# syun88/VLA-from-FastVLM

Hardware: AMD Instinct MI355X
Metric: policy steps/sec (img+prompt->action) FastVLM-0.5B bs=64 (higher is better)
Workload: dtype bf16; 1 GPU; fastvlm-0.5b select_action: letterbox 336^2->1024^2, FastViT-HD, projector, Qwen2 decoder (text-only, reference-literal: 64-token prompt), last-token pool, action head; batch_per_gpu=64, global_batch=64, seq_len=64, image=336, parallelism=replicas x1 (no collective on the inference path), tower_microbatch=0, stream_overlap=True, llm_precision=split-bf16 (hi+lo) operands, fp32 attention

## Files before the change

### vla-from-fastvlm_amd/csrc/decoder_kernels.hip

```cpp
#include "kernels.h"

namespace fv {
#define FV_TRY_RC(expr) do { const int rc_ = (expr); if (rc_ != FV_OK) return rc_; } while (0)
namespace {

__global__ __launch_bounds__(256) void embed_gather_kernel(const int32_t* __restrict__ ids,
                                                            const bf16_t* __restrict__ table,
                                                            const float* __restrict__ img, float* __restrict__ x, int T,
                                                            int Ni, int H, int vocab, long rows) {
  const int lane = threadIdx.x & 63;
  const long row = (long)blockIdx.x * 4 + (threadIdx.x >> 6);
  if (row >= rows) return;
  const int Tt = Ni + T;
  const long b = row / Tt;
  const int t = (int)(row % Tt);
  float* dst = x + row * H;
  if (t < Ni) {
    const float* src = img + (b * Ni + t) * H;
    for (int i = lane * 4; i < H; i += 256) *reinterpret_cast<float4*>(dst + i) = *reinterpret_cast<const float4*>(src + i);
  } else {
    int id = ids[b * T + (t - Ni)];
    id = min(max(id, 0), vocab - 1);
    const bf16_t* src = table + (size_t)id * H;
    for (int i = lane * 8; i < H; i += 512) {
// ... 353 lines not shown
  const float denom = mode == 0 ? 1.0f : fmaxf((float)(r1 - r0), 1e-6f);
  for (int i = tid; i < H; i += 256) pooled[(size_t)b * H + i] = 0.f;
  for (int r = r0; r < r1; ++r) {
    const float* xr = x + ((size_t)b * Ttot + r) * H;
    float ss = 0.f;
    for (int i = tid; i < H; i += 256) ss += xr[i] * xr[i];
    ss = wave_sum(ss);
    __syncthreads();
    if ((tid & 63) == 0) red[tid >> 6] = ss;
    __syncthreads();
    const float rs = rsqrtf((red[0] + red[1] + red[2] + red[3]) / (float)H + eps);
    for (int i = tid; i < H; i += 256) pooled[(size_t)b * H + i] += w[i] * (xr[i] * rs) / denom;
  }
}

}

int launch_embed_gather(const int32_t* ids, const bf16_t* table, const float* img_tokens, float* x, int B, int T,
                        int Ni, int H, int vocab, hipStream_t s) {
  if (!ids || !table || !x) return fv_fail(FV_ERR_ARG, "embed_gather: null pointer");
  if (Ni > 0 && !img_tokens) return fv_fail(FV_ERR_ARG, "embed_gather: Ni > 0 without image tokens");
  if (B <= 0 || T <= 0 || Ni < 0 || H % 8 || vocab <= 0) return fv_fail(FV_ERR_ARG, "embed_gather: bad shape");
  const long rows = (long)B * (Ni + T);
  hipLaunchKernelGGL(embed_gather_kernel, dim3((unsigned)((rows + 3) / 4)), dim3(256), 0, s, ids, table, img_tokens, x, T, Ni, H, vocab, rows);
  FV_HIP_CHECK(hipGetLastError());
  return FV_OK;
}

int launch_rmsnorm(const float* x, const float* w, bf16_t* y, bf16_t* y_lo, int ldy, int rows, int H, float eps, hipStream_t s, int f16, unsigned* sat, int lo8) {
  if (!x || !w || !y) return fv_fail(FV_ERR_ARG, "rmsnorm: null pointer");
// ... 149 lines not shown
```

### vla-from-fastvlm_amd/csrc/engine.hip

```cpp
#include <dlfcn.h>

#include <algorithm>
#include <exception>
#include <climits>
#include <cmath>
#include <new>
#include <cstdarg>
#include <cstdio>
#include <cstdlib>
#include <cstring>
#include <functional>
#include <map>
#include <string>
#include <vector>

#include "kernels.h"

static thread_local char g_err[768] = "";
static thread_local char* g_err_handle = nullptr;
int fv_fail(int code, const char* fmt, ...) {
  va_list ap;
  va_start(ap, fmt);
  vsnprintf(g_err, sizeof(g_err), fmt, ap);
  va_end(ap);
// ... 584 lines not shown
  }
  const int CL = d.tower_dims[d.tower_stages - 1], CO = d.tower_out_dim, P = H * H;
  FV_P(FV_FAM_DWCONV, dw_flops(mb, H, H, CO, 3), 2.0 * mb * P * (CL + CO), fv::launch_dwconv(cur, tw.exp_w, tw.exp_b, oth, mb, H, H, CL, 3, 1, CO / CL, 0, s));
  FV_P(FV_FAM_ELT, 20.0 * mb * P * CO, 6.0 * mb * P * CO, fv::launch_se_gelu(oth, tw.se_w1, tw.se_b1, tw.se_w2, tw.se_b2, tower_out, se, mb, P, CO, d.tower_se_rd, s));
  fv::GemmArgs p0{tower_out, CO, tw.pj0_w, mb * P, d.llm_hidden, CO, tw.pj0_b, nullptr, nullptr, 0, hid, d.llm_hidden, FV_EPI_BIAS_GELU};
  if (!h->batch_invariant) { p0.splitk_ws = h->ffn_part; p0.splitk_bytes = h->ffn_part ? FFN_PART_BYTES : 0; }
  FV_TRY(gemm_p(h, p0, s));
  fv::GemmArgs p2{hid, d.llm_hidden, tw.pj2_w, mb * P, d.llm_hidden, d.llm_hidden, tw.pj2_b, nullptr, nullptr, 0, img_tokens, d.llm_hidden, FV_EPI_F32};
  FV_TRY(gemm_p(h, p2, s));
  return FV_OK;
}


enum DecMode { DEC_FULL = 0, DEC_PREFIX = 1, DEC_SUFFIX = 2 };
int decoder_layers_split(fv_handle* h, const WsPlan& wp, int B, int Tq, const int32_t* lens, int len_add, float* kv, int Np, int mode,
                         hipStream_t s) {
  const fv_model_desc& d = h->d;
  char* ws = static_cast<char*>(h->ws);
  float* x = reinterpret_cast<float*>(ws + wp.x);
  bf16_t* xn = reinterpret_cast<bf16_t*>(ws + wp.xn);
  bf16_t* act = reinterpret_cast<bf16_t*>(ws + wp.act);
  const int rows = B * Tq, Hd = d.llm_hidden, D = d.llm_head_dim;
  const int qd = d.llm_heads * D, kd = d.llm_kv_heads * D, qkvw = qd + 2 * kd;
  const int Tt = mode == DEC_SUFFIX ? Np + Tq : Tq;
  const float att_scale = 1.0f / std::sqrt((float)D);
  {
    bf16_t* xs = reinterpret_cast<bf16_t*>(ws + wp.xn_lo);
    bf16_t* as = reinterpret_cast<bf16_t*>(ws + wp.att_lo);
    bf16_t* cs = reinterpret_cast<bf16_t*>(ws + wp.act_lo);
    float* qkvf = reinterpret_cast<float*>(ws + wp.qkvf);
    const int I = d.llm_inter, I2 = 2 * I;
// ... 4 lines not shown
      if (li == 0) FV_P(FV_FAM_NORM, 4.0 * rows * Hd, 8.0 * rows * Hd, fv::launch_rmsnorm(x, L.ln1, xs, xs + Hd, 2 * Hd, rows, Hd, d.rms_eps, s, 0, nullptr, lo8));
      fv::GemmArgs q1{xs, 2 * Hd, L.qkv_w, rows, qkvw, Hd, L.qkv_b, nullptr, nullptr, 0, qkvf, qkvw, FV_EPI_F32, KS};
      q1.W8 = L.qkv_w8;
      q1.splitk_ws = wp.splitk_bytes ? reinterpret_cast<float*>(ws + wp.splitk) : nullptr;
      q1.splitk_bytes = wp.splitk_bytes;
      FV_TRY(gemm_p(h, q1, s));
      if (mode == DEC_PREFIX) {
        FV_HIP_CHECK(hipMemcpy2DAsync(kv + li * kv_layer, (size_t)2 * kd * 4, qkvf + qd, (size_t)qkvw * 4, (size_t)2 * kd * 4, (size_t)rows,
                                      hipMemcpyDeviceToDevice, s));
        if (li + 1 == h->dec.layers.size()) break;
      }
      FV_P(FV_FAM_ATTN, 2.0 * B * (double)Tq * Tt * qd + 3.0 * rows * (qd + kd), 4.0 * rows * (qkvw + qd),
           fv::launch_attention_f32(qkvf, qkvw, as, as + qd, 2 * qd, B, Tt, d.llm_heads, d.llm_kv_heads, D, lens, len_add, att_scale, s, h->rope,
                                    mode == DEC_SUFFIX ? kv + li * kv_layer : nullptr, 2 * kd, mode == DEC_SUFFIX ? Np : 0, nullptr, lo8,
                                    wp.attn_scr_bytes && mode != DEC_SUFFIX ? ws + wp.attn_scr : nullptr));
      fv::GemmArgs o1{as, 2 * qd, L.o_w, rows, Hd, qd, nullptr, nullptr, x, Hd, x, Hd, FV_EPI_RES_F32, KS};
      o1.W8 = L.o_w8;
      o1.splitk_ws = q1.splitk_ws;
      o1.splitk_bytes = wp.splitk_bytes;
      const bool ln2_fused = d.llm_precision == 1 || d.llm_precision == 5;
      if (ln2_fused) { o1.norm_w = L.ln2; o1.norm_y = xs; o1.norm_ylo = xs + Hd; o1.norm_ld = 2 * Hd; o1.norm_eps = d.rms_eps; }
      FV_TRY(gemm_p(h, o1, s));
      fv::GemmArgs d1{cs, I2, L.down_w, rows, Hd, I, nullptr, nullptr, x, Hd, x, Hd, FV_EPI_RES_F32, KS};
      d1.W8 = L.down_w8;
      if (d.llm_precision == 2) {
        FV_P(FV_FAM_NORM, 4.0 * rows * Hd, 6.0 * rows * Hd, fv::launch_rmsnorm(x, L.ln2, xn, nullptr, Hd, rows, Hd, d.rms_eps, s, 1, h->f16_flags));
        fv::GemmArgs g1{xn, Hd, L.gu_w, rows, I2, Hd, nullptr, nullptr, nullptr, 0, act, I, FV_EPI_SWIGLU_F16, 0};
        g1.f16 = 1; g1.sat = h->f16_flags;
        FV_TRY(gemm_p(h, g1, s));
        d1 = fv::GemmArgs{act, I, L.down_w, rows, Hd, I, nullptr, nullptr, x, Hd, x, Hd, FV_EPI_RES_F32, 0};
// ... 414 lines not shown
      fv::GemmArgs gq{xn, Hd, L.qkv_w, rows, qkvw, Hd, L.qkv_b, nullptr, nullptr, 0, qkv, qkvw, FV_EPI_BIAS};
      FV_TRY(gemm_p(h, gq, s));
      FV_P(FV_FAM_ELT, 3.0 * rows * (qd + kd), 4.0 * rows * (qd + kd), fv::launch_rope(qkv, h->rope, qkvw, rows, Tt, d.llm_heads, d.llm_kv_heads, D, s));
      FV_P(FV_FAM_ATTN, 2.0 * B * (double)Tt * Tt * qd, 2.0 * rows * (qkvw + qd),
           fv::launch_attention(qkv, qkv + qd, qkv + qd + kd, qkvw, qkvw, qkvw, att, qd, B, Tt, d.llm_heads, d.llm_kv_heads,
                                D, 1, lens, Ni, att_scale, s));
      fv::GemmArgs go{att, qd, L.o_w, rows, Hd, qd, nullptr, nullptr, x, Hd, x, Hd, FV_EPI_RES_F32};
      FV_TRY(gemm_p(h, go, s));
      FV_P(FV_FAM_NORM, 4.0 * rows * Hd, 6.0 * rows * Hd, fv::launch_rmsnorm(x, L.ln2, xn, nullptr, Hd, rows, Hd, d.rms_eps, s));
      fv::GemmArgs gg{xn, Hd, L.gu_w, rows, 2 * d.llm_inter, Hd, nullptr, nullptr, nullptr, 0, act, d.llm_inter, FV_EPI_SWIGLU};
      FV_TRY(gemm_p(h, gg, s));
      fv::GemmArgs gd{act, d.llm_inter, L.down_w, rows, Hd, d.llm_inter, nullptr, nullptr, x, Hd, x, Hd, FV_EPI_RES_F32};
      FV_TRY(gemm_p(h, gd, s));
    }
  } else {
    FV_TRY(decoder_layers_split(h, wp, B, Tt, lens, Ni, nullptr, 0, DEC_FULL, s));
  }
  FV_P(FV_FAM_ELT, 4.0 * B * Hd, 8.0 * B * Hd, fv::launch_pool_norm(x, lens, h->dec.norm, static_cast<float*>(pooled), B, Tt, Ni, Hd, d.rms_eps, pool_mode, s));
  return FV_OK;
}

int fv_set_batch_invariant(fv_handle* h, int on) {
  HandleScope _hs(h);
  if (!h) return fv_fail(FV_ERR_ARG, "fv_set_batch_invariant: null handle");
  h->batch_invariant = on != 0;
  return FV_OK;
}

int fv_llm_fp16_saturations(fv_handle* h, uint64_t* count_out, int reset) {
  HandleScope _hs(h);
  if (!h || !count_out) return fv_fail(FV_ERR_ARG, "fv_llm_fp16_saturations: null argument");
// ... 33 lines not shown
                                   int pool_mode, void* pooled, fv_stream st) {
  HandleScope _hs(h);
  FV_TRY(check_ready(h, true));
  if (!ids || !lens || !kv || !pooled || B <= 0 || T <= 0 || Ni <= 0) return fv_fail(FV_ERR_ARG, "fv_llm_forward_pooled_prefixed: bad argument");
  const fv_model_desc& d = h->d;
  if (d.llm_precision == 0 || d.llm_head_dim < 64) return fv_fail(FV_ERR_UNSUPPORTED, "fv_llm_forward_pooled_prefixed: needs llm_precision 1 / 2 and head_dim 64 / 128");
  if (pool_mode != 0) return fv_fail(FV_ERR_UNSUPPORTED, "fv_llm_forward_pooled_prefixed: mean_pool averages the image positions too, which this pass does not recompute");
  if (T + Ni > h->rope_rows) return fv_fail(FV_ERR_ARG, "sequence of %d tokens exceeds the RoPE table (%d)", T + Ni, h->rope_rows);
  if (B > d.max_batch) return fv_fail(FV_ERR_ARG, "B=%d exceeds max_batch=%d", B, d.max_batch);
  const WsPlan wp = plan_ws(h, B, T, 1);
  if (wp.total > h->ws_bytes) return fv_fail(FV_ERR_STATE, "workspace too small (%zu > %zu)", wp.total, h->ws_bytes);
  hipStream_t s = static_cast<hipStream_t>(st);
  float* x = reinterpret_cast<float*>(static_cast<char*>(h->ws) + wp.x);
  const int Hd = d.llm_hidden;
  FV_P(FV_FAM_ELT, 0.0, 6.0 * B * T * Hd, fv::launch_embed_gather(ids, h->dec.embed, nullptr, x, B, T, 0, Hd, d.llm_vocab, s));
  FV_TRY(decoder_layers_split(h, wp, B, T, lens, Ni, const_cast<float*>(static_cast<const float*>(kv)), Ni, DEC_SUFFIX, s));
  FV_P(FV_FAM_ELT, 4.0 * B * Hd, 8.0 * B * Hd, fv::launch_pool_norm(x, lens, h->dec.norm, static_cast<float*>(pooled), B, T, 0, Hd, d.rms_eps, 0, s));
  return FV_OK;
}

int fv_head_layout(fv_handle* h, int64_t offsets[13]) {
  HandleScope _hs(h);
  if (!h || !offsets) return fv_fail(FV_ERR_ARG, "fv_head_layout: null argument");
  const fv::HeadOffsets ho = fv::head_offsets(h->hd);
  for (int i = 0; i < 13; ++i) offsets[i] = ho.o[i];
  return FV_OK;
}

int fv_head_saved_bytes(fv_handle* h, int B, size_t* out_bytes) {
  HandleScope _hs(h);
  if (!h || !out_bytes || B <= 0) return fv_fail(FV_ERR_ARG, "fv_head_saved_bytes: bad argument");
  *out_bytes = fv::head_saved_bytes(h->hd, B);
// ... 286 lines not shown
```

### vla-from-fastvlm_amd/csrc/gemm_bf16.hip

```cpp
#include <cstdlib>
#include <type_traits>

#include "kernels.h"

namespace fv {
namespace {

constexpr int BN = 128, BK = 64;
constexpr int LDC = BN + 4;

struct Params {
  const bf16_t* A; const bf16_t* W; const float* bias; const float* scale; const void* res; void* out;
  int M, N, K, lda, ldr, ldo, epi, tiles_n, nwg, ksplit;
  int splits = 1, npad = 0; float* part = nullptr;
  int lo_off = 0;
  int tiles_m = 0;
  int group_m = 0, tiles_mt = 0;
  int ldw = 0;
  const uint8_t* W8 = nullptr;
  unsigned* sat = nullptr;
  void* stash = nullptr;
  int stash_f16 = 0;
};

// ... 283 lines not shown
#define G2_T(I) { const unsigned long long n_ = __builtin_readcyclecounter(); st_[I] += n_ - t0_; t0_ = n_; }
#else
#define G2_T(I)
#endif
typedef __attribute__((address_space(3))) void* lds_ptr_t;
typedef const __attribute__((address_space(1))) void* gptr_t;
typedef __attribute__((ext_vector_type(4))) short g2_s16x4;
__device__ __forceinline__ bf16x8 g2_tr_frag(const char* region, int cols16, int c16, int ks, uint32_t tr_lane, int fq_hi) {
  const char* p0 = region + ((((4 * ks + fq_hi) * (cols16 >> 2) + (c16 >> 2)) << 10) + (((c16 >> 1) & 1) << 9) + ((c16 & 1) << 5) + tr_lane);
  const g2_s16x4 lo = __builtin_amdgcn_ds_read_tr16_b64_v4i16((g2_s16x4 __attribute__((address_space(3)))*)(p0));
  const g2_s16x4 hi = __builtin_amdgcn_ds_read_tr16_b64_v4i16((g2_s16x4 __attribute__((address_space(3)))*)(p0 + ((2 * (cols16 >> 2)) << 10)));
  const uint2 lu = __builtin_bit_cast(uint2, lo), hu = __builtin_bit_cast(uint2, hi);
  return __builtin_bit_cast(bf16x8, make_uint4(lu.x, lu.y, hu.x, hu.y));
}

template <int MI, int WN, bool ASYM = false, bool F16 = false, bool LO8 = false, bool TN = false>
__global__ __launch_bounds__(128 * WN, WN == 4 ? 1 : 2) void gemm256_kernel(Params p) {
  static_assert(!ASYM || WN == 4, "asymmetric staging pairs wave w with wave w + 4");
  static_assert(!TN || (!ASYM && !LO8 && MI == 8 && WN == 4), "the TN instance is the plain 256 x 256 one");
  constexpr int BMT = 32 * MI, BNT = 64 * WN, NTH = 128 * WN, BUFB = (BMT + BNT) * 128, AB = BMT * 128;
  constexpr int SA = BMT * 8 / NTH, SW = BNT * 8 / NTH;
  static_assert(SA * NTH == BMT * 8 && SW * NTH == BNT * 8 && SA <= 4 && SW <= 4, "whole slots per thread");
  extern __shared__ __attribute__((aligned(16))) char g2_smem[];
  const int tid = threadIdx.x, lane = tid & 63, wid = tid >> 6;
  const int wr = wid / WN, wc = wid % WN;
  const int fr = lane & 15, fq = lane >> 4;
  const int nk1 = p.K / BK, nk = LO8 ? nk1 + p.K / 128 : (p.ksplit ? 2 * nk1 : nk1);
#ifdef FASTVLA_AB_SWITCHES
  const int krot = (g_g2_krot && !p.ksplit && p.splits == 1) ? (int)((blockIdx.x * 13u) % (unsigned)nk) : 0;
  auto a_boff = [&](int kt0_) { const int kt = krot ? (kt0_ + krot) % nk : kt0_; if constexpr (TN) return kt * BK * p.lda * 2; else return LO8 && kt >= nk1 ? 2 * p.K + (kt - nk1) * 128 : ((kt >= nk1 ? kt - nk1 : kt) * BK + (kt >= nk1 ? p.K : 0)) * 2; };
  auto w_boff = [&](int kt0_) { const int kt = krot ? (kt0_ + krot) % nk : kt0_; if constexpr (TN) return kt * BK * p.ldw * 2; else return LO8 && kt >= nk1 ? (kt - nk1) * 128 : (kt >= nk1 ? kt - nk1 : kt) * BK * 2; };
#else
  auto a_boff = [&](int kt) { if constexpr (TN) return kt * BK * p.lda * 2; else return LO8 && kt >= nk1 ? 2 * p.K + (kt - nk1) * 128 : ((kt >= nk1 ? kt - nk1 : kt) * BK + (kt >= nk1 ? p.K : 0)) * 2; };
  auto w_boff = [&](int kt) { if constexpr (TN) return kt * BK * p.ldw * 2; else return LO8 && kt >= nk1 ? (kt - nk1) * 128 : (kt >= nk1 ? kt - nk1 : kt) * BK * 2; };
#endif
  const int wslot = __builtin_amdgcn_readfirstlane(wid) * 1024;

  uint32_t offa[4], offw[4], offa_n[4], offw_n[4];
  uint32_t offw2[4] = {0u, 0u, 0u, 0u}, offw2_n[4] = {0u, 0u, 0u, 0u};
  const int a32 = 32 * p.lda * 2;
  auto tile_offsets = [&](int unit, uint32_t (&oa)[4], uint32_t (&ow)[4], uint32_t (&ow2)[4], int& bm, int& bn) {
    const int logical = xcd_remap(unit, p.nwg) / p.splits;
// ... 41 lines not shown
        for (int j = 0; j < SA; ++j) {
          __builtin_amdgcn_raw_ptr_buffer_load_lds(arsrc, (lds_ptr_t)(la + j * (NTH * 16)), 16, oa[j], aoff, 0, 0);
          __builtin_amdgcn_raw_ptr_buffer_load_lds(arsrc, (lds_ptr_t)(la + j * (NTH * 16) + 4096), 16, oa[j], aoff + a32, 0, 0);
        }
#pragma unroll
        for (int j = 0; j < SW; ++j) {
          __builtin_amdgcn_raw_ptr_buffer_load_lds(wrsrc, (lds_ptr_t)(lw + j * (NTH * 16)), 16, ow[j], woff, 0, 0);
          __builtin_amdgcn_raw_ptr_buffer_load_lds(wrsrc, (lds_ptr_t)(lw + j * (NTH * 16) + 4096), 16, ow2[j], woff, 0, 0);
        }
      }
    } else {
#pragma unroll
      for (int j = 0; j < SA; ++j) __builtin_amdgcn_raw_ptr_buffer_load_lds(arsrc, (lds_ptr_t)(la + j * (NTH * 16)), 16, oa[j], aoff, 0, 0);
#pragma unroll
      for (int j = 0; j < SW; ++j) __builtin_amdgcn_raw_ptr_buffer_load_lds(wrsrc, (lds_ptr_t)(lw + j * (NTH * 16)), 16, ow[j], woff, 0, 0);
    }
  };
  const uint32_t tr_lane = (uint32_t)((4 * (fq & 1) + (fr >> 2)) * 64 + (fr & 3) * 8);
  const uint32_t fo0 = (uint32_t)(fr * 128 + (((0 * 4 + fq) ^ (fr & 7)) << 4));
  const uint32_t fo1 = (uint32_t)(fr * 128 + (((1 * 4 + fq) ^ (fr & 7)) << 4));

  int tile = blockIdx.x, pb = 0, bm, bn, bm_n = 0, bn_n = 0;
  if (tile >= p.nwg) return;
  tile_offsets(tile, offa, offw, offw2, bm, bn);
  auto k_lo = [&](int unit) { return (xcd_remap(unit, p.nwg) % p.splits) * nk / p.splits; };
  auto k_hi = [&](int unit) { return (xcd_remap(unit, p.nwg) % p.splits + 1) * nk / p.splits; };
  stage(offa, offw, offw2, k_lo(tile), 0);
  asm volatile("s_waitcnt vmcnt(0)" ::: "memory");
  __syncthreads();
#ifdef G2_STAMPS
  unsigned long long st_[8] = {0, 0, 0, 0, 0, 0, 0, 0}, t0_ = __builtin_readcyclecounter();
#endif
  for (; tile < p.nwg; tile += (int)gridDim.x) {
    const int next = tile + (int)gridDim.x;
    if (next < p.nwg) tile_offsets(next, offa_n, offw_n, offw2_n, bm_n, bn_n);
    const int kt0 = k_lo(tile), kt1 = k_hi(tile), kn0 = next < p.nwg ? k_lo(next) : 0;
    f32x4 acc[4][MI];
#pragma unroll
    for (int j = 0; j < 4; ++j)
#pragma unroll
      for (int i = 0; i < MI; ++i) acc[j][i] = f32x4{0.f, 0.f, 0.f, 0.f};
    auto ktile = [&](auto f8_tag, int kt) {
      constexpr bool F8T = decltype(f8_tag)::value;
        const int cur = (pb + kt - kt0) & 1;
        G2_T(4)
        const bool st_same = kt + 1 < kt1, st_any = st_same || next < p.nwg;
  #if G2_DEAL
        const int st_kt = st_same ? kt + 1 : kn0;
        const int st_aoff = a_boff(st_kt), st_woff = w_boff(st_kt);
        const __amdgpu_buffer_rsrc_t wrsrc = LO8 && st_kt >= nk1 ? wrsrc_f8 : wrsrc_bf;
        char* st_la = g2_smem + (cur ^ 1) * BUFB + wslot;
        char* st_lw = st_la + AB;
  #else
        if (st_same) stage(offa, offw, offw2, kt + 1, cur ^ 1);
        else if (st_any) stage(offa_n, offw_n, offw2_n, kn0, cur ^ 1);
  #endif
        G2_T(0)
        const char* la = g2_smem + cur * BUFB + (wr * (16 * MI)) * 128;
        const char* lw = g2_smem + cur * BUFB + AB + (wc * 64) * 128;
        if constexpr (F8T) {
          i32x8 w8f[4], x8f[2];
  #define G2_RD8(BASE, T) ld_f8op((BASE) + (T) * 2048 + fo0, (BASE) + (T) * 2048 + fo1)
  #pragma unroll
          for (int j = 0; j < 4; ++j) w8f[j] = G2_RD8(lw, j);
          x8f[0] = G2_RD8(la, 0);
  #pragma unroll
          for (int t = 0; t < MI; ++t) {
            if (t + 1 < MI) x8f[(t + 1) & 1] = G2_RD8(la, t + 1);
  #if G2_DEAL
            if (t < SA + SW && st_any) {
              if (t < SA) __builtin_amdgcn_raw_ptr_buffer_load_lds(arsrc, (lds_ptr_t)(st_la + (t % 4) * (NTH * 16)), 16, st_same ? offa[t % 4] : offa_n[t % 4], st_aoff, 0, 0);
              else __builtin_amdgcn_raw_ptr_buffer_load_lds(wrsrc, (lds_ptr_t)(st_lw + ((t - SA) % 4) * (NTH * 16)), 16, st_same ? offw[(t - SA) % 4] : offw_n[(t - SA) % 4], st_woff, 0, 0);
            }
  #endif
  #pragma unroll
            for (int j = 0; j < 4; ++j) acc[j][t] = mfma_lo8(w8f[j], x8f[t & 1], acc[j][t]);
            __builtin_amdgcn_sched_barrier(0);
          }
  #undef G2_RD8
        } else {
          bf16x8 fwA[4], fwB[4], far[3];
  #define G2_RD_A(T) (TN ? g2_tr_frag(g2_smem + cur * BUFB, BMT / 16, wr * MI + (T) % MI, (T) / MI, tr_lane, fq >> 1) \
                         : __builtin_bit_cast(bf16x8, *reinterpret_cast<const uint4*>(la + ((T) % MI) * 2048 + ((T) / MI ? fo1 : fo0))))
  #define G2_RD_W(KS, J) (TN ? g2_tr_frag(g2_smem + cur * BUFB + AB, BNT / 16, wc * 4 + (J), (KS), tr_lane, fq >> 1) \
                             : __builtin_bit_cast(bf16x8, *reinterpret_cast<const uint4*>(lw + (J) * 2048 + ((KS) ? fo1 : fo0))))
  #pragma unroll
          for (int j = 0; j < 4; ++j) fwA[j] = G2_RD_W(0, j);
          far[0] = G2_RD_A(0);
          far[1] = G2_RD_A(1);
  #pragma unroll
          for (int t = 0; t < 2 * MI; ++t) {
            if (t + 2 < 2 * MI) far[(t + 2) % 3] = G2_RD_A(t + 2);
  #if G2_DEAL
            if (t < SA + SW && st_any) {
              if (t < SA) __builtin_amdgcn_raw_ptr_buffer_load_lds(arsrc, (lds_ptr_t)(st_la + (t % 4) * (NTH * 16)), 16, st_same ? offa[t % 4] : offa_n[t % 4], st_aoff, 0, 0);
              else __builtin_amdgcn_raw_ptr_buffer_load_lds(wrsrc, (lds_ptr_t)(st_lw + ((t - SA) % 4) * (NTH * 16)), 16, st_same ? offw[(t - SA) % 4] : offw_n[(t - SA) % 4], st_woff, 0, 0);
            }
  #endif
            if (t == MI - 3) {
  #pragma unroll
              for (int j = 0; j < 4; ++j) fwB[j] = G2_RD_W(1, j);
            }
  #pragma unroll
            for (int j = 0; j < 4; ++j)
              acc[j][t % MI] = mfma16<F16>(t < MI ? fwA[j] : fwB[j], far[t % 3], acc[j][t % MI]);
            __builtin_amdgcn_sched_barrier(0);
          }
  #undef G2_RD_A
  #undef G2_RD_W
        }
        G2_T(1)
        asm volatile("s_waitcnt vmcnt(0)" ::: "memory");
        G2_T(2)
        __syncthreads();
        G2_T(3)
  #ifdef G2_STAMPS
        st_[6] += 1;
  #endif
    };
    {
      const int kmid = LO8 ? (kt1 < nk1 ? kt1 : nk1) : kt1;
      for (int kt = kt0; kt < kmid; ++kt) ktile(std::false_type{}, kt);
      if constexpr (LO8) for (int kt = kt0 > nk1 ? kt0 : nk1; kt < kt1; ++kt) ktile(std::true_type{}, kt);
    }

    constexpr int ORB = 64 * 4 + 16;
    if constexpr (LO8) lo8_settle();
    char* so = g2_smem + ((pb + kt1 - kt0 - 1) & 1) * BUFB + wid * (16 * ORB);
    const int c8 = lane & 7;
    const int gn = bn + wc * 64 + c8 * 8;
    float bs[8], sc[8];
#pragma unroll
    for (int e = 0; e < 8; ++e) { bs[e] = 0.f; sc[e] = 1.f; }
    const bool col_ok = gn < p.N;
    if (p.bias && p.splits == 1 && col_ok) {
      const float4 lo = *reinterpret_cast<const float4*>(p.bias + gn), hi = *reinterpret_cast<const float4*>(p.bias + gn + 4);
      bs[0] = lo.x; bs[1] = lo.y; bs[2] = lo.z; bs[3] = lo.w; bs[4] = hi.x; bs[5] = hi.y; bs[6] = hi.z; bs[7] = hi.w;
    }
    if (p.epi == FV_EPI_LS_RES && col_ok) {
      const float4 lo = *reinterpret_cast<const float4*>(p.scale + gn), hi = *reinterpret_cast<const float4*>(p.scale + gn + 4);
      sc[0] = lo.x; sc[1] = lo.y; sc[2] = lo.z; sc[3] = lo.w; sc[4] = hi.x; sc[5] = hi.y; sc[6] = hi.z; sc[7] = hi.w;
    }
#pragma unroll
// ... 529 lines not shown
    if (a.f16) return fv_fail(FV_ERR_ARG, "gemm: hi + lo8 goes with bf16 hi operands");
  } else if (a.ksplit && a.lda < 2 * a.K) return fv_fail(FV_ERR_ARG, "gemm: ksplit needs lda >= 2K");
  static int cus = 0;
  if (!cus) {
    int dev = 0;
    hipDeviceProp_t prop;
    cus = (hipGetDevice(&dev) == hipSuccess && hipGetDeviceProperties(&prop, dev) == hipSuccess && prop.multiProcessorCount > 0) ? prop.multiProcessorCount : 256;
    FV_HIP_CHECK(hipFuncSetAttribute(reinterpret_cast<const void*>(&gemm256_kernel<8, 4>), hipFuncAttributeMaxDynamicSharedMemorySize, 2 * 512 * 128));
    FV_HIP_CHECK(hipFuncSetAttribute(reinterpret_cast<const void*>(&gemm256_kernel<4, 2>), hipFuncAttributeMaxDynamicSharedMemorySize, 2 * 256 * 128));
    FV_HIP_CHECK(hipFuncSetAttribute(reinterpret_cast<const void*>(&gemm256_kernel<8, 4, true>), hipFuncAttributeMaxDynamicSharedMemorySize, 2 * 512 * 128));
    FV_HIP_CHECK(hipFuncSetAttribute(reinterpret_cast<const void*>(&gemm256_kernel<8, 4, false, true>), hipFuncAttributeMaxDynamicSharedMemorySize, 2 * 512 * 128));
    FV_HIP_CHECK(hipFuncSetAttribute(reinterpret_cast<const void*>(&gemm256_kernel<8, 4, true, true>), hipFuncAttributeMaxDynamicSharedMemorySize, 2 * 512 * 128));
    FV_HIP_CHECK(hipFuncSetAttribute(reinterpret_cast<const void*>(&gemm256_kernel<8, 4, false, false, true>), hipFuncAttributeMaxDynamicSharedMemorySize, 2 * 512 * 128));
    FV_HIP_CHECK(hipFuncSetAttribute(reinterpret_cast<const void*>(&gemm256_kernel<4, 2, false, false, true>), hipFuncAttributeMaxDynamicSharedMemorySize, 2 * 256 * 128));
    FV_HIP_CHECK(hipFuncSetAttribute(reinterpret_cast<const void*>(&gemm256_kernel<4, 2, false, true>), hipFuncAttributeMaxDynamicSharedMemorySize, 2 * 256 * 128));
  }
  static const bool colmajor_ok = fv_ab_env("FASTVLA_NO_GEMM_COLMAJOR") == nullptr;
  constexpr int cm_max = 8;
  static const bool no_asym = fv_ab_env("FASTVLA_NO_GEMM_ASYM") != nullptr;
  static const int min_kt_per_range = fv_ab_env("FASTVLA_GEMM_MIN_KT") ? atoi(fv_ab_env("FASTVLA_GEMM_MIN_KT")) : 16;
  static const int group_m_default = fv_ab_env("FASTVLA_GEMM_GROUP_M") ? atoi(fv_ab_env("FASTVLA_GEMM_GROUP_M")) : 4;
  const bool asym = !no_asym && a.M <= 8192 && a.M % 256 == 0;
  static const bool no_tail_env = fv_ab_env("FASTVLA_NO_GEMM_TAIL") != nullptr;
  if (!no_tail_env && !a.no_tail && a.few_rows && a.splitk_ws && !a.norm_w && !a.stash && !a.f16 && a.ksplit != 2 && a.M % 256 == 0 && a.N % 256 == 0 &&
      a.K % 64 == 0 && (f32out || (a.epi == FV_EPI_SWIGLU_SPLIT && a.N % 512 == 0)) && gemm_glds_tile(a) == 256) {
    const int tmr = a.M / 256, tn = a.N / 256, tiles = tmr * tn, rem = tiles % cus, nkt = (a.ksplit ? 2 : 1) * (a.K / 64);
    if (tiles > cus && rem > 0 && 2 * rem <= cus && rem % tmr == 0 && nkt >= 32) {
      const int n0 = (tn - rem / tmr) * 256;
      const int lo = a.lo_off ? a.lo_off : a.N / 2;
      GemmArgs a1 = a, a2 = a;
      a1.N = n0; a1.no_tail = 1; a1.lo_off = lo;
      a2.N = a.N - n0; a2.no_tail = 1; a2.lo_off = lo;
      a2.W = a.W + (size_t)n0 * a.K;
      if (a.bias) a2.bias = a.bias + n0;
      if (f32out) {
        a2.out = static_cast<float*>(a.out) + n0;
        if (a.res) a2.res = static_cast<const float*>(a.res) + n0;
// ... 43 lines not shown
      splits = tiles < cus ? cus / tiles : 1;
      if (splits > 8) splits = 8;
      while (splits > 1 && nkt / splits < 16) --splits;
      while (splits > 1 && (size_t)splits * a.M * (tn * 256) * sizeof(float) > a.splitk_bytes) --splits;
    } else {
      const double tile_us = (double)nkt * 64.0 * 131072.0 / 1.0e6 / 4.0;
      const double part_us = 2.0 * (double)a.M * (tn * 256) * 4.0 / 4.0e6;
      double best = 1e30;
      for (int sN = 1; sN <= 8; ++sN) {
        if (sN > 1 && (nkt / sN < min_kt_per_range || (size_t)sN * a.M * (tn * 256) * sizeof(float) > a.splitk_bytes)) break;
        const long units = (long)tiles * sN, rounds = (units + cus - 1) / cus;
        const double t = (double)rounds * tile_us / sN + (sN > 1 ? sN * part_us : 0.0);
        if (t < best * 0.97) { best = t; splits = sN; }
      }
    }
    if (splits > 1) {
      p.tiles_n = tn;
      p.tiles_m = colmajor_ok && tmr <= cm_max ? tmr : 0;
      p.tiles_mt = tmr; p.group_m = (!p.tiles_m && tn > 8) ? pick_group_m(tmr, group_m_default) : 0;
      p.splits = splits; p.npad = tn * 256; p.part = a.splitk_ws;
      p.nwg = tiles * splits;
      const dim3 g2(p.nwg < cus ? p.nwg : cus / 8 * 8);
       if (a.ksplit == 2) hipLaunchKernelGGL((gemm256_kernel<8, 4, false, false, true>), g2, dim3(512), 2 * 512 * 128, s, p);
      else if (a.f16 && asym) hipLaunchKernelGGL((gemm256_kernel<8, 4, true, true>), g2, dim3(512), 2 * 512 * 128, s, p);
      else if (a.f16) hipLaunchKernelGGL((gemm256_kernel<8, 4, false, true>), g2, dim3(512), 2 * 512 * 128, s, p);
      else if (asym) hipLaunchKernelGGL((gemm256_kernel<8, 4, true>), g2, dim3(512), 2 * 512 * 128, s, p);
      else hipLaunchKernelGGL((gemm256_kernel<8, 4>), g2, dim3(512), 2 * 512 * 128, s, p);
      return launch_splitk_reduce(a, splits, p.npad, false, a.ksplit == 2 ? 1 : 0, s);
    }
  }
  static const bool no_pw = fv_ab_env("FASTVLA_NO_PWCONV") != nullptr;
  if (!no_pw && !a.ksplit && !a.f16 && a.N == a.K && (a.K == 96 || a.K == 192) && a.lda == a.K && a.ldo == a.N && a.M % 128 == 0 &&
      (a.epi == FV_EPI_BIAS || a.epi == FV_EPI_BIAS_GELU)) {
    const int tiles = a.M / 128;
    if (a.K == 96) {
      constexpr int LDS = 96 * (96 * 2 + 16) + 4 * 32 * (96 * 2 + 16);
      static bool set96 = false;
      if (!set96) { FV_HIP_CHECK(hipFuncSetAttribute(reinterpret_cast<const void*>(&pwconv_kernel<96>), hipFuncAttributeMaxDynamicSharedMemorySize, LDS)); set96 = true; }
      hipLaunchKernelGGL(pwconv_kernel<96>, dim3(tiles < 3 * cus ? tiles : 3 * cus), dim3(256), LDS, s, p);
    } else {
// ... 6 lines not shown
    return FV_OK;
  }
  if (const int gt = gemm_glds_tile(a)) {
    const int tmr = (a.M + gt - 1) / gt;
    p.tiles_n = (a.N + gt - 1) / gt;
    p.nwg = tmr * p.tiles_n;
    p.tiles_m = colmajor_ok && tmr <= cm_max ? tmr : 0;
    p.tiles_mt = tmr; p.group_m = (!p.tiles_m && p.tiles_n > 8) ? pick_group_m(tmr, group_m_default) : 0;
    int slots = (gt == 128 ? 2 * cus : cus) / 8 * 8;
    if (const char* e = fv_ab_env("FASTVLA_GEMM_GRID")) { const int v = atoi(e); if (v >= 8 && gt == 256) slots = v / 8 * 8; }
    const int grid = p.nwg < slots ? p.nwg : slots;
    if (gt == 256 && a.ksplit == 2) hipLaunchKernelGGL((gemm256_kernel<8, 4, false, false, true>), dim3(grid), dim3(512), 2 * 512 * 128, s, p);
    else if (a.ksplit == 2) hipLaunchKernelGGL((gemm256_kernel<4, 2, false, false, true>), dim3(grid), dim3(256), 2 * 256 * 128, s, p);
    else if (gt == 256 && a.f16 && asym) hipLaunchKernelGGL((gemm256_kernel<8, 4, true, true>), dim3(grid), dim3(512), 2 * 512 * 128, s, p);
    else if (gt == 256 && a.f16) hipLaunchKernelGGL((gemm256_kernel<8, 4, false, true>), dim3(grid), dim3(512), 2 * 512 * 128, s, p);
    else if (gt == 256 && asym) hipLaunchKernelGGL((gemm256_kernel<8, 4, true>), dim3(grid), dim3(512), 2 * 512 * 128, s, p);
    else if (gt == 256) hipLaunchKernelGGL((gemm256_kernel<8, 4>), dim3(grid), dim3(512), 2 * 512 * 128, s, p);
    else if (a.f16) hipLaunchKernelGGL((gemm256_kernel<4, 2, false, true>), dim3(grid), dim3(256), 2 * 256 * 128, s, p);
    else hipLaunchKernelGGL((gemm256_kernel<4, 2>), dim3(grid), dim3(256), 2 * 256 * 128, s, p);
    FV_HIP_CHECK(hipGetLastError());
    return FV_OK;
  }
  p.tiles_n = (a.N + BN - 1) / BN;
  const long blocks128 = (long)((a.M + 127) / 128) * p.tiles_n;
  if (blocks128 >= 512) {
    p.nwg = (int)blocks128;
    if (a.ksplit == 2) hipLaunchKernelGGL((gemm_kernel<128, false, true>), dim3(p.nwg), dim3(256), 0, s, p);
    else if (a.f16) hipLaunchKernelGGL((gemm_kernel<128, true>), dim3(p.nwg), dim3(256), 0, s, p);
    else hipLaunchKernelGGL(gemm_kernel<128>, dim3(p.nwg), dim3(256), 0, s, p);
  } else {
    p.nwg = ((a.M + 63) / 64) * p.tiles_n;
    if (a.ksplit == 2) hipLaunchKernelGGL((gemm_kernel<64, false, true>), dim3(p.nwg), dim3(256), 0, s, p);
// ... 13 lines not shown
```

### vla-from-fastvlm_amd/csrc/kernels.h

```cpp
#pragma once
#include <hip/hip_runtime.h>
#include <stdint.h>

#include "../../include/fastvla_hip.h"
#include "../../include/fastvla_hip_testops.h"
#include "common.h"

namespace fv {

struct GemmArgs {
  const bf16_t* A; int lda;
  const bf16_t* W;
  int M, N, K;
  const float* bias;
  const float* scale;
  const void* res; int ldr;
  void* out; int ldo;
  int epi;
  int ksplit = 0;
  int f16 = 0;
  float* splitk_ws = nullptr;
  size_t splitk_bytes = 0;
  int lo_off = 0;
  int no_tail = 0;
// ... 63 lines not shown
int launch_bf16_to_f16(bf16_t* p, size_t n, float scale, hipStream_t s, unsigned* maxbits = nullptr);
int launch_bf16_to_w8(const bf16_t* w, void* w8, size_t rows, int K, hipStream_t s, unsigned* maxbits = nullptr);
int launch_rope_f32(float* qkv, const float2* table, int ld, int rows, int T, int heads, int kv_heads, int D, hipStream_t s);
int launch_attention_f32(float* qkv, int ld, bf16_t* out_hi, bf16_t* out_lo, int ldo, int B, int T, int heads,
                         int kv_heads, int D, const int32_t* lens, int len_add, float scale, hipStream_t s, const float2* rope = nullptr,
                         const float* pre = nullptr, int ldp = 0, int Np = 0,
                         float* lse = nullptr,
                         int lo8 = 0,
                         void* split_scratch = nullptr);
constexpr int FV_ATTN_SPLIT_MIN_T = 128;
int launch_rope(bf16_t* qkv, const float2* table, int ld, int rows, int T, int heads, int kv_heads, int D,
                hipStream_t s);
void rope_table_host(float* cos_sin_pairs, int T, int D, float theta);
int launch_pool_norm(const float* x, const int32_t* lens, const float* w, float* pooled, int B, int Ttot, int Ni,
                     int H, float eps, int mode, hipStream_t s);

constexpr int RMS_BWD_RPW = 4;
constexpr int COLSUM_CHUNKS = 64;
int launch_split_rows(const float* in, int ldi, bf16_t* out, int ldo, int lo_off, long R, int C, hipStream_t s);
int launch_lo8_rows(const float* in, int ldi, bf16_t* out, int ldo, long R, int C, hipStream_t s);
int launch_bf16_to_f32(const bf16_t* in, float* out, size_t n, hipStream_t s);
int launch_transpose_to_bf16(const void* in, int in_bf16, int ldi, bf16_t* out, int ldo, int lo_off, int R, int Rp, int C, hipStream_t s);
int launch_transpose_to_f16(const void* in, int in_kind, int ldi, int lo_in, bf16_t* out, int ldo, int R, int Rp, int C, unsigned* sat, hipStream_t s,
                            bf16_t* rows_out = nullptr, int ldro = 0);
int launch_rows_to_f16(const void* in, int in_kind, int ldi, int lo_in, bf16_t* out, int ldo, long R, int C, unsigned* sat, hipStream_t s,
                       long Rp = 0);
int launch_swiglu_bwd(float* gu, const float* dact, long rows, int I, hipStream_t s, bf16_t* out_split = nullptr);
int launch_swiglu_bwd_rows(const void* gu, int gu_f16, const float* dact, long rows, long Rp, int I, bf16_t* dgu_rows, bf16_t* act_rows, unsigned* sat, hipStream_t s);
int launch_swiglu_bwd_f16(const void* gu, int gu_f16, const float* dact, int rows, int Rp, int I, bf16_t* out_rows, bf16_t* outT, unsigned* sat, hipStream_t s,
                          bf16_t* actT = nullptr);
// ... 138 lines not shown
```

Baseline: 19.14 steps/s.

## Compute last decoder layer only for pooled rows; add paired hi/lo GEMM k-walk

When pooling takes only the last token, the final decoder layer's o-proj, norm, gate-up and down GEMMs now run on just the B gathered rows instead of all B*T rows. A new gather kernel copies the attention output and residual for each sample's last valid row into scratch that reuses the qkv buffer. Separately, a PAIRED variant of the 256-tile GEMM interleaves the hi and lo bf16 operand k-tiles in one loop: W tiles are staged once and shared by both A halves, with the lo A half going to the other buffer. This variant is used whenever ksplit==1 and the op is not fp16, which adds new staging and buffer-index logic that could be wrong or change pipelining.

```diff
diff --git a/vla-from-fastvlm_amd/csrc/decoder_kernels.hip b/vla-from-fastvlm_amd/csrc/decoder_kernels.hip
--- a/vla-from-fastvlm_amd/csrc/decoder_kernels.hip
+++ b/vla-from-fastvlm_amd/csrc/decoder_kernels.hip
@@ -391,6 +391,27 @@
   }
 }
 
+__global__ __launch_bounds__(256) void gather_pool_rows_kernel(const uint4* __restrict__ att, const uint4* __restrict__ x, const int32_t* __restrict__ lens,
+                                                                uint4* __restrict__ att_c, uint4* __restrict__ x_c, int Tq, int Ni, int att_q, int x_q) {
+  const int b = blockIdx.x, tid = threadIdx.x;
+  int len = lens ? lens[b] : (Tq - Ni);
+  len = min(max(len, 0), Tq - Ni);
+  const size_t r = (size_t)b * Tq + Ni + max(len - 1, 0);
+  for (int i = tid; i < att_q; i += 256) att_c[(size_t)b * att_q + i] = att[r * att_q + i];
+  for (int i = tid; i < x_q; i += 256) x_c[(size_t)b * x_q + i] = x[r * x_q + i];
+}
+
+}
+
+int launch_gather_pool_rows(const bf16_t* att, int att_cols, const float* x, int H, const int32_t* lens, bf16_t* att_c, float* x_c, int B, int Tq, int Ni,
+                            hipStream_t s) {
+  if (!att || !x || !att_c || !x_c) return fv_fail(FV_ERR_ARG, "gather_pool_rows: null pointer");
+  if (B <= 0 || Tq <= Ni || Ni < 0 || att_cols <= 0 || att_cols % 8 || H <= 0 || H % 4) return fv_fail(FV_ERR_ARG, "gather_pool_rows: bad shape");
+  if (((uintptr_t)att | (uintptr_t)x | (uintptr_t)att_c | (uintptr_t)x_c) & 15) return fv_fail(FV_ERR_ARG, "gather_pool_rows: pointers must be 16-byte aligned");
+  hipLaunchKernelGGL(gather_pool_rows_kernel, dim3(B), dim3(256), 0, s, reinterpret_cast<const uint4*>(att), reinterpret_cast<const uint4*>(x), lens,
+                     reinterpret_cast<uint4*>(att_c), reinterpret_cast<uint4*>(x_c), Tq, Ni, att_cols / 8, H / 4);
+  FV_HIP_CHECK(hipGetLastError());
+  return FV_OK;
 }
 
 int launch_embed_gather(const int32_t* ids, const bf16_t* table, const float* img_tokens, float* x, int B, int T,
diff --git a/vla-from-fastvlm_amd/csrc/engine.hip b/vla-from-fastvlm_amd/csrc/engine.hip
--- a/vla-from-fastvlm_amd/csrc/engine.hip
+++ b/vla-from-fastvlm_amd/csrc/engine.hip
@@ -622,7 +622,7 @@
 
 enum DecMode { DEC_FULL = 0, DEC_PREFIX = 1, DEC_SUFFIX = 2 };
 int decoder_layers_split(fv_handle* h, const WsPlan& wp, int B, int Tq, const int32_t* lens, int len_add, float* kv, int Np, int mode,
-                         hipStream_t s) {
+                         hipStream_t s, int pool_mode = 1, const float** x_pool = nullptr) {
   const fv_model_desc& d = h->d;
   char* ws = static_cast<char*>(h->ws);
   float* x = reinterpret_cast<float*>(ws + wp.x);
@@ -657,6 +657,29 @@
            fv::launch_attention_f32(qkvf, qkvw, as, as + qd, 2 * qd, B, Tt, d.llm_heads, d.llm_kv_heads, D, lens, len_add, att_scale, s, h->rope,
                                     mode == DEC_SUFFIX ? kv + li * kv_layer : nullptr, 2 * kd, mode == DEC_SUFFIX ? Np : 0, nullptr, lo8,
                                     wp.attn_scr_bytes && mode != DEC_SUFFIX ? ws + wp.attn_scr : nullptr));
+      const size_t compact_bytes = (size_t)B * (4 * (size_t)qd + 8 * (size_t)Hd + 4 * (size_t)I);
+      if (x_pool && pool_mode == 0 && mode != DEC_PREFIX && li + 1 == h->dec.layers.size() && (d.llm_precision == 1 || lo8) && Tq > 1 &&
+          compact_bytes <= (size_t)rows * qkvw * 4) {
+        bf16_t* asc = reinterpret_cast<bf16_t*>(qkvf);
+        float* xc = reinterpret_cast<float*>(asc + (size_t)B * 2 * qd);
+        bf16_t* xsc = reinterpret_cast<bf16_t*>(xc + (size_t)B * Hd);
+        bf16_t* csc = xsc + (size_t)B * 2 * Hd;
+        FV_P(FV_FAM_ELT, 0.0, 2.0 * B * (4.0 * qd + 4.0 * Hd),
+             fv::launch_gather_pool_rows(as, 2 * qd, x, Hd, lens, asc, xc, B, Tq, mode == DEC_FULL ? len_add : 0, s));
+        float* skw = wp.splitk_bytes ? reinterpret_cast<float*>(ws + wp.splitk) : nullptr;
+        fv::GemmArgs oc{asc, 2 * qd, L.o_w, B, Hd, qd, nullptr, nullptr, xc, Hd, xc, Hd, FV_EPI_RES_F32, KS};
+        oc.W8 = L.o_w8; oc.splitk_ws = skw; oc.splitk_bytes = wp.splitk_bytes;
+        oc.norm_w = L.ln2; oc.norm_y = xsc; oc.norm_ylo = xsc + Hd; oc.norm_ld = 2 * Hd; oc.norm_eps = d.rms_eps;
+        FV_TRY(gemm_p(h, oc, s));
+        fv::GemmArgs gc{xsc, 2 * Hd, L.gu_w, B, I2, Hd, nullptr, nullptr, nullptr, 0, csc, I2, FV_EPI_SWIGLU_SPLIT, KS};
+        gc.W8 = L.gu_w8; gc.splitk_ws = skw; gc.splitk_bytes = wp.splitk_bytes;
+        FV_TRY(gemm_p(h, gc, s));
+        fv::GemmArgs dc{csc, I2, L.down_w, B, Hd, I, nullptr, nullptr, xc, Hd, xc, Hd, FV_EPI_RES_F32, KS};
+        dc.W8 = L.down_w8; dc.splitk_ws = skw; dc.splitk_bytes = wp.splitk_bytes;
+        FV_TRY(gemm_p(h, dc, s));
+        *x_pool = xc;
+        break;
+      }
       fv::GemmArgs o1{as, 2 * qd, L.o_w, rows, Hd, qd, nullptr, nullptr, x, Hd, x, Hd, FV_EPI_RES_F32, KS};
       o1.W8 = L.o_w8;
       o1.splitk_ws = q1.splitk_ws;
@@ -1101,7 +1124,12 @@
       FV_TRY(gemm_p(h, gd, s));
     }
   } else {
-    FV_TRY(decoder_layers_split(h, wp, B, Tt, lens, Ni, nullptr, 0, DEC_FULL, s));
+    const float* xc = nullptr;
+    FV_TRY(decoder_layers_split(h, wp, B, Tt, lens, Ni, nullptr, 0, DEC_FULL, s, pool_mode, &xc));
+    if (xc) {
+      FV_P(FV_FAM_ELT, 4.0 * B * Hd, 8.0 * B * Hd, fv::launch_pool_norm(xc, nullptr, h->dec.norm, static_cast<float*>(pooled), B, 1, 0, Hd, d.rms_eps, 0, s));
+      return FV_OK;
+    }
   }
   FV_P(FV_FAM_ELT, 4.0 * B * Hd, 8.0 * B * Hd, fv::launch_pool_norm(x, lens, h->dec.norm, static_cast<float*>(pooled), B, Tt, Ni, Hd, d.rms_eps, pool_mode, s));
   return FV_OK;
@@ -1165,8 +1193,10 @@
   float* x = reinterpret_cast<float*>(static_cast<char*>(h->ws) + wp.x);
   const int Hd = d.llm_hidden;
   FV_P(FV_FAM_ELT, 0.0, 6.0 * B * T * Hd, fv::launch_embed_gather(ids, h->dec.embed, nullptr, x, B, T, 0, Hd, d.llm_vocab, s));
-  FV_TRY(decoder_layers_split(h, wp, B, T, lens, Ni, const_cast<float*>(static_cast<const float*>(kv)), Ni, DEC_SUFFIX, s));
-  FV_P(FV_FAM_ELT, 4.0 * B * Hd, 8.0 * B * Hd, fv::launch_pool_norm(x, lens, h->dec.norm, static_cast<float*>(pooled), B, T, 0, Hd, d.rms_eps, 0, s));
+  const float* xc = nullptr;
+  FV_TRY(decoder_layers_split(h, wp, B, T, lens, Ni, const_cast<float*>(static_cast<const float*>(kv)), Ni, DEC_SUFFIX, s, 0, &xc));
+  if (xc) FV_P(FV_FAM_ELT, 4.0 * B * Hd, 8.0 * B * Hd, fv::launch_pool_norm(xc, nullptr, h->dec.norm, static_cast<float*>(pooled), B, 1, 0, Hd, d.rms_eps, 0, s));
+  else FV_P(FV_FAM_ELT, 4.0 * B * Hd, 8.0 * B * Hd, fv::launch_pool_norm(x, lens, h->dec.norm, static_cast<float*>(pooled), B, T, 0, Hd, d.rms_eps, 0, s));
   return FV_OK;
 }
 
diff --git a/vla-from-fastvlm_amd/csrc/gemm_bf16.hip b/vla-from-fastvlm_amd/csrc/gemm_bf16.hip
--- a/vla-from-fastvlm_amd/csrc/gemm_bf16.hip
+++ b/vla-from-fastvlm_amd/csrc/gemm_bf16.hip
@@ -321,9 +321,10 @@
   return __builtin_bit_cast(bf16x8, make_uint4(lu.x, lu.y, hu.x, hu.y));
 }
 
-template <int MI, int WN, bool ASYM = false, bool F16 = false, bool LO8 = false, bool TN = false>
+template <int MI, int WN, bool ASYM = false, bool F16 = false, bool LO8 = false, bool TN = false, bool PAIRED = false>
 __global__ __launch_bounds__(128 * WN, WN == 4 ? 1 : 2) void gemm256_kernel(Params p) {
   static_assert(!ASYM || WN == 4, "asymmetric staging pairs wave w with wave w + 4");
+  static_assert(!PAIRED || (!F16 && !LO8 && !TN), "the paired walk is the bf16 hi | lo form's");
   static_assert(!TN || (!ASYM && !LO8 && MI == 8 && WN == 4), "the TN instance is the plain 256 x 256 one");
   constexpr int BMT = 32 * MI, BNT = 64 * WN, NTH = 128 * WN, BUFB = (BMT + BNT) * 128, AB = BMT * 128;
   constexpr int SA = BMT * 8 / NTH, SW = BNT * 8 / NTH;
@@ -332,7 +333,7 @@
   const int tid = threadIdx.x, lane = tid & 63, wid = tid >> 6;
   const int wr = wid / WN, wc = wid % WN;
   const int fr = lane & 15, fq = lane >> 4;
-  const int nk1 = p.K / BK, nk = LO8 ? nk1 + p.K / 128 : (p.ksplit ? 2 * nk1 : nk1);
+  const int nk1 = p.K / BK, nk = PAIRED ? nk1 : LO8 ? nk1 + p.K / 128 : (p.ksplit ? 2 * nk1 : nk1);
 #ifdef FASTVLA_AB_SWITCHES
   const int krot = (g_g2_krot && !p.ksplit && p.splits == 1) ? (int)((blockIdx.x * 13u) % (unsigned)nk) : 0;
   auto a_boff = [&](int kt0_) { const int kt = krot ? (kt0_ + krot) % nk : kt0_; if constexpr (TN) return kt * BK * p.lda * 2; else return LO8 && kt >= nk1 ? 2 * p.K + (kt - nk1) * 128 : ((kt >= nk1 ? kt - nk1 : kt) * BK + (kt >= nk1 ? p.K : 0)) * 2; };
@@ -404,6 +405,36 @@
       for (int j = 0; j < SA; ++j) __builtin_amdgcn_raw_ptr_buffer_load_lds(arsrc, (lds_ptr_t)(la + j * (NTH * 16)), 16, oa[j], aoff, 0, 0);
 #pragma unroll
       for (int j = 0; j < SW; ++j) __builtin_amdgcn_raw_ptr_buffer_load_lds(wrsrc, (lds_ptr_t)(lw + j * (NTH * 16)), 16, ow[j], woff, 0, 0);
+    }
+  };
+  auto stage_a = [&](const uint32_t (&oa)[4], int aoff, int abuf) {
+    char* la = g2_smem + abuf * BUFB + wslot;
+    if constexpr (ASYM) {
+      if (wr == 0) {
+#pragma unroll
+        for (int j = 0; j < SA; ++j) {
+          __builtin_amdgcn_raw_ptr_buffer_load_lds(arsrc, (lds_ptr_t)(la + j * (NTH * 16)), 16, oa[j], aoff, 0, 0);
+          __builtin_amdgcn_raw_ptr_buffer_load_lds(arsrc, (lds_ptr_t)(la + j * (NTH * 16) + 4096), 16, oa[j], aoff + a32, 0, 0);
+        }
+      }
+    } else {
+#pragma unroll
+      for (int j = 0; j < SA; ++j) __builtin_amdgcn_raw_ptr_buffer_load_lds(arsrc, (lds_ptr_t)(la + j * (NTH * 16)), 16, oa[j], aoff, 0, 0);
+    }
+  };
+  auto stage_w = [&](const uint32_t (&ow)[4], const uint32_t (&ow2)[4], int woff, int wbuf) {
+    char* lw = g2_smem + wbuf * BUFB + AB + wslot;
+    if constexpr (ASYM) {
+      if (wr == 0) {
+#pragma unroll
+        for (int j = 0; j < SW; ++j) {
+          __builtin_amdgcn_raw_ptr_buffer_load_lds(wrsrc_bf, (lds_ptr_t)(lw + j * (NTH * 16)), 16, ow[j], woff, 0, 0);
+          __builtin_amdgcn_raw_ptr_buffer_load_lds(wrsrc_bf, (lds_ptr_t)(lw + j * (NTH * 16) + 4096), 16, ow2[j], woff, 0, 0);
+        }
+      }
+    } else {
+#pragma unroll
+      for (int j = 0; j < SW; ++j) __builtin_amdgcn_raw_ptr_buffer_load_lds(wrsrc_bf, (lds_ptr_t)(lw + j * (NTH * 16)), 16, ow[j], woff, 0, 0);
     }
   };
   const uint32_t tr_lane = (uint32_t)((4 * (fq & 1) + (fr >> 2)) * 64 + (fr & 3) * 8);
@@ -432,9 +463,21 @@
       for (int i = 0; i < MI; ++i) acc[j][i] = f32x4{0.f, 0.f, 0.f, 0.f};
     auto ktile = [&](auto f8_tag, int kt) {
       constexpr bool F8T = decltype(f8_tag)::value;
-        const int cur = (pb + kt - kt0) & 1;
+        const int cur = PAIRED ? (pb + (kt >> 1) - kt0) & 1 : (pb + kt - kt0) & 1;
+        const int abuf = PAIRED ? kt & 1 : cur;
         G2_T(4)
-        const bool st_same = kt + 1 < kt1, st_any = st_same || next < p.nwg;
+        const bool st_same = (PAIRED ? (kt >> 1) + 1 : kt + 1) < kt1, st_any = st_same || next < p.nwg;
+        if constexpr (PAIRED) {
+          if (!(kt & 1)) stage_a(offa, ((kt >> 1) * BK + p.K) * 2, 1);
+          else if (st_any) {
+            uint32_t oa_[4], ow_[4], ow2_[4];
+#pragma unroll
+            for (int j = 0; j < 4; ++j) { oa_[j] = st_same ? offa[j] : offa_n[j]; ow_[j] = st_same ? offw[j] : offw_n[j]; ow2_[j] = st_same ? offw2[j] : offw2_n[j]; }
+            const int koff = (st_same ? (kt >> 1) + 1 : kn0) * BK * 2;
+            stage_a(oa_, koff, 0);
+            stage_w(ow_, ow2_, koff, cur ^ 1);
+          }
+        }
   #if G2_DEAL
         const int st_kt = st_same ? kt + 1 : kn0;
         const int st_aoff = a_boff(st_kt), st_woff = w_boff(st_kt);
@@ -442,11 +485,13 @@
         char* st_la = g2_smem + (cur ^ 1) * BUFB + wslot;
         char* st_lw = st_la + AB;
   #else
-        if (st_same) stage(offa, offw, offw2, kt + 1, cur ^ 1);
-        else if (st_any) stage(offa_n, offw_n, offw2_n, kn0, cur ^ 1);
+        if constexpr (!PAIRED) {
+          if (st_same) stage(offa, offw, offw2, kt + 1, cur ^ 1);
+          else if (st_any) stage(offa_n, offw_n, offw2_n, kn0, cur ^ 1);
+        }
   #endif
         G2_T(0)
-        const char* la = g2_smem + cur * BUFB + (wr * (16 * MI)) * 128;
+        const char* la = g2_smem + abuf * BUFB + (wr * (16 * MI)) * 128;
         const char* lw = g2_smem + cur * BUFB + AB + (wc * 64) * 128;
         if constexpr (F8T) {
           i32x8 w8f[4], x8f[2];
@@ -458,7 +503,7 @@
           for (int t = 0; t < MI; ++t) {
             if (t + 1 < MI) x8f[(t + 1) & 1] = G2_RD8(la, t + 1);
   #if G2_DEAL
-            if (t < SA + SW && st_any) {
+            if (!PAIRED && t < SA + SW && st_any) {
               if (t < SA) __builtin_amdgcn_raw_ptr_buffer_load_lds(arsrc, (lds_ptr_t)(st_la + (t % 4) * (NTH * 16)), 16, st_same ? offa[t % 4] : offa_n[t % 4], st_aoff, 0, 0);
               else __builtin_amdgcn_raw_ptr_buffer_load_lds(wrsrc, (lds_ptr_t)(st_lw + ((t - SA) % 4) * (NTH * 16)), 16, st_same ? offw[(t - SA) % 4] : offw_n[(t - SA) % 4], st_woff, 0, 0);
             }
@@ -482,7 +527,7 @@
           for (int t = 0; t < 2 * MI; ++t) {
             if (t + 2 < 2 * MI) far[(t + 2) % 3] = G2_RD_A(t + 2);
   #if G2_DEAL
-            if (t < SA + SW && st_any) {
+            if (!PAIRED && t < SA + SW && st_any) {
               if (t < SA) __builtin_amdgcn_raw_ptr_buffer_load_lds(arsrc, (lds_ptr_t)(st_la + (t % 4) * (NTH * 16)), 16, st_same ? offa[t % 4] : offa_n[t % 4], st_aoff, 0, 0);
               else __builtin_amdgcn_raw_ptr_buffer_load_lds(wrsrc, (lds_ptr_t)(st_lw + ((t - SA) % 4) * (NTH * 16)), 16, st_same ? offw[(t - SA) % 4] : offw_n[(t - SA) % 4], st_woff, 0, 0);
             }
@@ -510,13 +555,16 @@
     };
     {
       const int kmid = LO8 ? (kt1 < nk1 ? kt1 : nk1) : kt1;
+      if constexpr (PAIRED) {
+        for (int kt = 2 * kt0; kt < 2 * kt1; ++kt) ktile(std::false_type{}, kt);
+      } else
       for (int kt = kt0; kt < kmid; ++kt) ktile(std::false_type{}, kt);
       if constexpr (LO8) for (int kt = kt0 > nk1 ? kt0 : nk1; kt < kt1; ++kt) ktile(std::true_type{}, kt);
     }
 
     constexpr int ORB = 64 * 4 + 16;
     if constexpr (LO8) lo8_settle();
-    char* so = g2_smem + ((pb + kt1 - kt0 - 1) & 1) * BUFB + wid * (16 * ORB);
+    char* so = g2_smem + (PAIRED ? (((pb + kt1 - kt0 - 1) & 1) ? BUFB : AB) : ((pb + kt1 - kt0 - 1) & 1) * BUFB) + wid * (16 * ORB);
     const int c8 = lane & 7;
     const int gn = bn + wc * 64 + c8 * 8;
     float bs[8], sc[8];
@@ -1076,6 +1124,9 @@
     FV_HIP_CHECK(hipFuncSetAttribute(reinterpret_cast<const void*>(&gemm256_kernel<8, 4, false, false, true>), hipFuncAttributeMaxDynamicSharedMemorySize, 2 * 512 * 128));
     FV_HIP_CHECK(hipFuncSetAttribute(reinterpret_cast<const void*>(&gemm256_kernel<4, 2, false, false, true>), hipFuncAttributeMaxDynamicSharedMemorySize, 2 * 256 * 128));
     FV_HIP_CHECK(hipFuncSetAttribute(reinterpret_cast<const void*>(&gemm256_kernel<4, 2, false, true>), hipFuncAttributeMaxDynamicSharedMemorySize, 2 * 256 * 128));
+    FV_HIP_CHECK(hipFuncSetAttribute(reinterpret_cast<const void*>(&gemm256_kernel<8, 4, false, false, false, false, true>), hipFuncAttributeMaxDynamicSharedMemorySize, 2 * 512 * 128));
+    FV_HIP_CHECK(hipFuncSetAttribute(reinterpret_cast<const void*>(&gemm256_kernel<8, 4, true, false, false, false, true>), hipFuncAttributeMaxDynamicSharedMemorySize, 2 * 512 * 128));
+    FV_HIP_CHECK(hipFuncSetAttribute(reinterpret_cast<const void*>(&gemm256_kernel<4, 2, false, false, false, false, true>), hipFuncAttributeMaxDynamicSharedMemorySize, 2 * 256 * 128));
   }
   static const bool colmajor_ok = fv_ab_env("FASTVLA_NO_GEMM_COLMAJOR") == nullptr;
   constexpr int cm_max = 8;
@@ -1083,6 +1134,8 @@
   static const int min_kt_per_range = fv_ab_env("FASTVLA_GEMM_MIN_KT") ? atoi(fv_ab_env("FASTVLA_GEMM_MIN_KT")) : 16;
   static const int group_m_default = fv_ab_env("FASTVLA_GEMM_GROUP_M") ? atoi(fv_ab_env("FASTVLA_GEMM_GROUP_M")) : 4;
   const bool asym = !no_asym && a.M <= 8192 && a.M % 256 == 0;
+  static const bool no_paired = fv_ab_env("FASTVLA_NO_GEMM_PAIRED") != nullptr;
+  const bool paired = !no_paired && p.ksplit == 1 && !a.f16;
   static const bool no_tail_env = fv_ab_env("FASTVLA_NO_GEMM_TAIL") != nullptr;
   if (!no_tail_env && !a.no_tail && a.few_rows && a.splitk_ws && !a.norm_w && !a.stash && !a.f16 && a.ksplit != 2 && a.M % 256 == 0 && a.N % 256 == 0 &&
       a.K % 64 == 0 && (f32out || (a.epi == FV_EPI_SWIGLU_SPLIT && a.N % 512 == 0)) && gemm_glds_tile(a) == 256) {
@@ -1156,6 +1209,7 @@
         if (t < best * 0.97) { best = t; splits = sN; }
       }
     }
+    if (paired && splits > a.K / 64) splits = a.K / 64;
     if (splits > 1) {
       p.tiles_n = tn;
       p.tiles_m = colmajor_ok && tmr <= cm_max ? tmr : 0;
@@ -1166,6 +1220,8 @@
        if (a.ksplit == 2) hipLaunchKernelGGL((gemm256_kernel<8, 4, false, false, true>), g2, dim3(512), 2 * 512 * 128, s, p);
       else if (a.f16 && asym) hipLaunchKernelGGL((gemm256_kernel<8, 4, true, true>), g2, dim3(512), 2 * 512 * 128, s, p);
       else if (a.f16) hipLaunchKernelGGL((gemm256_kernel<8, 4, false, true>), g2, dim3(512), 2 * 512 * 128, s, p);
+      else if (paired && asym) hipLaunchKernelGGL((gemm256_kernel<8, 4, true, false, false, false, true>), g2, dim3(512), 2 * 512 * 128, s, p);
+      else if (paired) hipLaunchKernelGGL((gemm256_kernel<8, 4, false, false, false, false, true>), g2, dim3(512), 2 * 512 * 128, s, p);
       else if (asym) hipLaunchKernelGGL((gemm256_kernel<8, 4, true>), g2, dim3(512), 2 * 512 * 128, s, p);
       else hipLaunchKernelGGL((gemm256_kernel<8, 4>), g2, dim3(512), 2 * 512 * 128, s, p);
       return launch_splitk_reduce(a, splits, p.npad, false, a.ksplit == 2 ? 1 : 0, s);
@@ -1202,8 +1258,11 @@
     else if (a.ksplit == 2) hipLaunchKernelGGL((gemm256_kernel<4, 2, false, false, true>), dim3(grid), dim3(256), 2 * 256 * 128, s, p);
     else if (gt == 256 && a.f16 && asym) hipLaunchKernelGGL((gemm256_kernel<8, 4, true, true>), dim3(grid), dim3(512), 2 * 512 * 128, s, p);
     else if (gt == 256 && a.f16) hipLaunchKernelGGL((gemm256_kernel<8, 4, false, true>), dim3(grid), dim3(512), 2 * 512 * 128, s, p);
+    else if (gt == 256 && paired && asym) hipLaunchKernelGGL((gemm256_kernel<8, 4, true, false, false, false, true>), dim3(grid), dim3(512), 2 * 512 * 128, s, p);
+    else if (gt == 256 && paired) hipLaunchKernelGGL((gemm256_kernel<8, 4, false, false, false, false, true>), dim3(grid), dim3(512), 2 * 512 * 128, s, p);
     else if (gt == 256 && asym) hipLaunchKernelGGL((gemm256_kernel<8, 4, true>), dim3(grid), dim3(512), 2 * 512 * 128, s, p);
     else if (gt == 256) hipLaunchKernelGGL((gemm256_kernel<8, 4>), dim3(grid), dim3(512), 2 * 512 * 128, s, p);
+    else if (paired) hipLaunchKernelGGL((gemm256_kernel<4, 2, false, false, false, false, true>), dim3(grid), dim3(256), 2 * 256 * 128, s, p);
     else if (a.f16) hipLaunchKernelGGL((gemm256_kernel<4, 2, false, true>), dim3(grid), dim3(256), 2 * 256 * 128, s, p);
     else hipLaunchKernelGGL((gemm256_kernel<4, 2>), dim3(grid), dim3(256), 2 * 256 * 128, s, p);
     FV_HIP_CHECK(hipGetLastError());
diff --git a/vla-from-fastvlm_amd/csrc/kernels.h b/vla-from-fastvlm_amd/csrc/kernels.h
--- a/vla-from-fastvlm_amd/csrc/kernels.h
+++ b/vla-from-fastvlm_amd/csrc/kernels.h
@@ -101,6 +101,8 @@
 void rope_table_host(float* cos_sin_pairs, int T, int D, float theta);
 int launch_pool_norm(const float* x, const int32_t* lens, const float* w, float* pooled, int B, int Ttot, int Ni,
                      int H, float eps, int mode, hipStream_t s);
+int launch_gather_pool_rows(const bf16_t* att, int att_cols, const float* x, int H, const int32_t* lens, bf16_t* att_c, float* x_c, int B, int Tq, int Ni,
+                            hipStream_t s);
 
 constexpr int RMS_BWD_RPW = 4;
 constexpr int COLSUM_CHUNKS = 64;
```

New measurement: 19.31 steps/s (median of 6 runs). No clear change (+0.9%).
